# nabeelre/BTSbot

Hardware: AMD Instinct MI355X
Metric: alerts/sec (63×63×3 triplet + 25 meta) train+infer, 1/2/4/8 MI355X (higher is better)
Workload: dtype bf16; 1 GPU; BASELINE.json configs[1]: ConvNeXt-pico multi-modal (mm_ConvNeXt) bf16 inference, batch=1024 synthetic triplets per GPU, inputs resident in HBM, logits+scores out; per_gpu_batch=1024, global_batch=1024, precision=bf16, weights=seeded random, layer-scale ~1, parallelism=1 independent replicas, batch-sharded, no collective, pipeline_depth=3

## Files before the change

### btsbot_amd/csrc/stage0b.hip

```cpp
#include <type_traits>

#include "common.h"
#include "stage0.h"

namespace {

typedef __attribute__((ext_vector_type(16))) float f32x16;
typedef __attribute__((address_space(1))) const void* gptr_t;
typedef __attribute__((address_space(3))) void* lptr_t;

template <typename T> struct SBM;
typedef __attribute__((ext_vector_type(4))) short s16x4;
typedef __attribute__((ext_vector_type(4))) _Float16 f16x4;
template <> struct SBM<bf16_t> {
  using frag = bf16x8;
  using frag4 = s16x4;
  static __device__ __forceinline__ f32x16 run(frag a, frag b, f32x16 c) {
    return __builtin_amdgcn_mfma_f32_32x32x16_bf16(a, b, c, 0, 0, 0);
  }
  static __device__ __forceinline__ f32x4 run4(frag4 a, frag4 b, f32x4 c) {
    return __builtin_amdgcn_mfma_f32_4x4x4bf16_1k(a, b, c, 0, 0, 0);
  }
};
template <> struct SBM<f16_t> {
  using frag = f16x8;
  using frag4 = f16x4;
  static __device__ __forceinline__ f32x16 run(frag a, frag b, f32x16 c) {
    return __builtin_amdgcn_mfma_f32_32x32x16_f16(a, b, c, 0, 0, 0);
  }
  static __device__ __forceinline__ f32x4 run4(frag4 a, frag4 b, f32x4 c) {
    return __builtin_amdgcn_mfma_f32_4x4x4f16(a, b, c, 0, 0, 0);
  }
};

constexpr int C = 64, HW = 15, P = 225, CT = 2, HID = 256;
constexpr int PITCH = 2 * C + 16;
static_assert(256 * PITCH <= C * 800, "the [pixel][channel] image overlays the planar one");
constexpr int PL_ROWS = 22, PL_XQ = PL_ROWS * 8, PL_CH = 800;
constexpr int PLB = C * PL_CH;
constexpr int CHUNKB = 8192, NCH = HID / 32, NSLOT = 3;
constexpr int RINGB = NSLOT * CHUNKB;
constexpr int TW_R = 21, TW_BYTES = TW_R * C * 4 * 4 * 2;
constexpr int PF_DWB = 0, PF_LNW = C, PF_LNB = 2 * C, PF_B1 = 3 * C, PF_B2 = PF_B1 + HID, PF_FLOATS = 512;
static_assert(PF_B2 + C == PF_FLOATS, "parameter image layout");
constexpr int PARB = TW_BYTES + PF_FLOATS * 4;
constexpr int PARB_X2 = 2 * TW_BYTES + PF_FLOATS * 4;
template <bool X2> struct S0L {
  static constexpr int PLANES = X2 ? 2 : 1;
  static constexpr int CHB = X2 ? 2 * CHUNKB : CHUNKB;
  static constexpr int OFF_RING = PLANES * PLB;
  static constexpr int OFF_B1 = OFF_RING + NSLOT * CHB;
  static constexpr int OFF_ST = OFF_B1 + (HID + C) * 4;
  static constexpr int LDS_BYTES = OFF_ST + 2 * 256 * 4;
};
static_assert(S0L<false>::LDS_BYTES <= 81920, "two workgroups per CU");
static_assert(S0L<true>::LDS_BYTES <= 160 * 1024, "one workgroup per CU");
constexpr float LN_EPS = 1e-6f;

#define SB_STAMP(i)                                                                \
  do {                                                                             \
    if (a.stamps != nullptr && blockIdx.x == 0 && threadIdx.x == 0) {             \
      a.stamps[i] = clock64();                                                     \
      asm volatile("s_waitcnt vmcnt(0)" ::: "memory");  \
    }                                                                              \
    if (a.wgt != nullptr && threadIdx.x == 0 && ((i) == 0 || (i) == 13))           \
      a.wgt[2 * blockIdx.x + ((i) == 13)] = wall_clock64();                        \
  } while (0)

struct __attribute__((packed, aligned(4))) f4u { float v[4]; };

template <int N> __device__ __forceinline__ void wait_vm() {
  asm volatile("s_waitcnt vmcnt(%0)" ::"n"(N) : "memory");
}
__device__ __forceinline__ int swz4(int row) {
  return (4 - ((row >> 2) & 3)) & 3;
}
__device__ __forceinline__ float swap_add32(float a, float b) {
  auto r = __builtin_amdgcn_permlane32_swap(__float_as_uint(a), __float_as_uint(b), false, false);
  return __uint_as_float(r[0]) + __uint_as_float(r[1]);
}
__device__ __forceinline__ float swap_add16(float a, float b) {
  auto r = __builtin_amdgcn_permlane16_swap(__float_as_uint(a), __float_as_uint(b), false, false);
  return __uint_as_float(r[0]) + __uint_as_float(r[1]);
}
__device__ __forceinline__ void ln_regs(const f32x16 (&x)[CT], const float* __restrict__ w,
                                        const float* __restrict__ b, int h, f32x16 (&y)[CT]) {
  float s = 0.f;
#pragma unroll
  for (int ct = 0; ct < CT; ++ct)
#pragma unroll
    for (int r = 0; r < 16; ++r) s += x[ct][r];
  s += __shfl_xor(s, 32, 64);
  const float mean = s * (1.0f / C);
  float q = 0.f;
#pragma unroll
  for (int ct = 0; ct < CT; ++ct)
#pragma unroll
    for (int r = 0; r < 16; ++r) {
      const float d = x[ct][r] - mean;
      q += d * d;
    }
  q += __shfl_xor(q, 32, 64);
  const float rstd = rsqrtf(q * (1.0f / C) + LN_EPS);
#pragma unroll
  for (int ct = 0; ct < CT; ++ct)
#pragma unroll
    for (int qd = 0; qd < 4; ++qd) {
      const int c = ct * 32 + 8 * qd + 4 * h;
      const float4 wv = *reinterpret_cast<const float4*>(w + c);
      const float4 bv = *reinterpret_cast<const float4*>(b + c);
      y[ct][4 * qd + 0] = (x[ct][4 * qd + 0] - mean) * rstd * wv.x + bv.x;
      y[ct][4 * qd + 1] = (x[ct][4 * qd + 1] - mean) * rstd * wv.y + bv.y;
      y[ct][4 * qd + 2] = (x[ct][4 * qd + 2] - mean) * rstd * wv.z + bv.z;
      y[ct][4 * qd + 3] = (x[ct][4 * qd + 3] - mean) * rstd * wv.w + bv.w;
    }
}

template <typename T, int LOPLANE = 0>
__device__ __forceinline__ void regs_to_map(const f32x16 (&x)[CT], unsigned char* map, int p, int h) {
  typedef T T4 __attribute__((ext_vector_type(4)));
#pragma unroll
  for (int ct = 0; ct < CT; ++ct)
#pragma unroll
    for (int qd = 0; qd < 4; ++qd) {
      T4 v, w;
#pragma unroll
      for (int e = 0; e < 4; ++e) {
        v[e] = (T)x[ct][4 * qd + e];
        if (LOPLANE > 0) w[e] = (T)(x[ct][4 * qd + e] - (float)v[e]);
      }
      *reinterpret_cast<T4*>(map + p * PITCH + (ct * 32 + 8 * qd + 4 * h) * 2) = v;
      if (LOPLANE > 0) *reinterpret_cast<T4*>(map + LOPLANE + p * PITCH + (ct * 32 + 8 * qd + 4 * h) * 2) = w;
    }
}

template <typename T, int LOPLANE = 0, bool SAT = false>
__device__ __forceinline__ void regs_to_planar(const f32x16 (&x)[CT], unsigned char* pl, int p, int h) {
  const int y = p / HW, xx = p - y * HW;
  unsigned char* dst = pl + (xx >> 2) * PL_XQ + (y + 3) * 8 + (xx & 3) * 2 + h * 4 * PL_CH;
#pragma unroll
  for (int ct = 0; ct < CT; ++ct)
#pragma unroll
    for (int r = 0; r < 16; ++r) {
      const T hi = (T)(SAT ? __builtin_amdgcn_fmed3f(x[ct][r], -65504.0f, 65504.0f) : x[ct][r]);
      *reinterpret_cast<T*>(dst + (ct * 32 + 8 * (r >> 2) + (r & 3)) * PL_CH) = hi;
      if (LOPLANE > 0)
        *reinterpret_cast<T*>(dst + LOPLANE + (ct * 32 + 8 * (r >> 2) + (r & 3)) * PL_CH) = (T)(x[ct][r] - (float)hi);
    }
}

__device__ __forceinline__ void regs_to_tap(const f32x16 (&x)[CT], float* tap, int h) {
#pragma unroll
  for (int ct = 0; ct < CT; ++ct)
#pragma unroll
    for (int qd = 0; qd < 4; ++qd)
      *reinterpret_cast<float4*>(tap + ct * 32 + 8 * qd + 4 * h) =
          make_float4(x[ct][4 * qd], x[ct][4 * qd + 1], x[ct][4 * qd + 2], x[ct][4 * qd + 3]);
}

template <int CTRL> __device__ __forceinline__ float dpp_mov(float v) {
  return __builtin_bit_cast(float, __builtin_amdgcn_update_dpp(0, __builtin_bit_cast(int, v), CTRL, 0xF, 0xF, true));
}

template <bool SQ> __device__ __forceinline__ void block_reduce64(const float (&v)[64], int lane, float (&out)[4]) {
  float w[32];
#pragma unroll
  for (int n = 0; n < 32; ++n)
    w[n] = SQ ? swap_add32(v[n] * v[n], v[n + 32] * v[n + 32]) : swap_add32(v[n], v[n + 32]);
#pragma unroll
  for (int n = 0; n < 16; ++n) w[n] = swap_add16(w[n], w[n + 16]);
  const bool b3 = (lane & 8) != 0, b2 = (lane & 4) != 0;
#pragma unroll
  for (int n = 0; n < 8; ++n) {
    const float own = b3 ? w[n + 8] : w[n], send = b3 ? w[n] : w[n + 8];
    w[n] = own + dpp_mov<0x128>(send);
  }
#pragma unroll
  for (int n = 0; n < 4; ++n) {
    const float own = b2 ? w[n + 4] : w[n], send = b2 ? w[n] : w[n + 4];
    const float lo = dpp_mov<0x124>(send), hi = dpp_mov<0x12C>(send);
    out[n] = own + (b2 ? lo : hi);
  }
}

template <typename T, bool X2, int WPS = 2, bool KEEP = false>
__global__ __launch_bounds__(256, WPS) void stage0b_kernel(Stage0Args a) {
  using frag = typename SBM<T>::frag;
  using DT = typename std::conditional<KEEP, f16_t, T>::type;
  using frag4 = typename SBM<DT>::frag4;
  extern __shared__ __attribute__((aligned(16))) unsigned char smem[];
  unsigned char* map = smem;
  unsigned char* pl = smem;
  using L = S0L<X2>;
  constexpr int CHB = L::CHB;
  constexpr int PLO = X2 ? PLB : 0;
  unsigned char* ring = smem + L::OFF_RING;
  float* b1s = reinterpret_cast<float*>(smem + L::OFF_B1);
  float* b2s = b1s + HID;
  float* part = reinterpret_cast<float*>(ring + 2 * CHB);
  float* st = reinterpret_cast<float*>(smem + L::OFF_ST);

  const int tid = threadIdx.x, lane = tid & 63, wave = tid >> 6;
  const int lr = lane & 31, h = lane >> 5;
  const int alert = blockIdx.x;
  int pix[2];
  bool live[2];
#pragma unroll
  for (int t = 0; t < 2; ++t) {
    pix[t] = wave * 64 + t * 32 + lr;
    live[t] = pix[t] < P;
  }
  const int dj = lane & 3, dch = wave * 16 + (lane >> 2);
  const int dyb = lane >> 4, dxb = (lane >> 2) & 3;

  SB_STAMP(0);
  frag4 tw[TW_R], twl[X2 ? TW_R : 1];
  float dwbias, lng, lnb2, b1v, b2v;
  auto load_block_params = [&](int j) {
    const Stage0Blk& bk = a.blk[j];
    const uint2* src = reinterpret_cast<const uint2*>(bk.par) + wave * 64 + lane;
#pragma unroll
    for (int r = 0; r < TW_R; ++r) tw[r] = __builtin_bit_cast(frag4, src[r * 256]);
    if (X2) {
#pragma unroll
      for (int r = 0; r < TW_R; ++r) twl[r] = __builtin_bit_cast(frag4, src[TW_BYTES / 8 + r * 256]);
    }
    const float* pf = reinterpret_cast<const float*>(bk.par + (X2 ? 2 : 1) * TW_BYTES);
    dwbias = pf[PF_DWB + dch];
    lng = pf[PF_LNW + dch];
    lnb2 = pf[PF_LNB + dch];
    b1v = pf[PF_B1 + tid];
    b2v = pf[PF_B2 + (tid & 63)];
  };
  load_block_params(0);
  auto zero_planar = [&]() {
    for (int i = tid; i < L::PLANES * PLB / 16; i += 256) reinterpret_cast<uint4*>(pl)[i] = make_uint4(0u, 0u, 0u, 0u);
  };
  zero_planar();
  __syncthreads();

  f32x16 x[2][CT];
  {
    const float* src = a.img + (size_t)alert * 3 * 63 * 63;
    const T* sw = reinterpret_cast<const T*>(a.stem_w);
    frag af[3][CT], afl[X2 ? 3 : 1][CT];
#pragma unroll
    for (int ci = 0; ci < 3; ++ci)
#pragma unroll
      for (int ct = 0; ct < CT; ++ct) {
        af[ci][ct] = *reinterpret_cast<const frag*>(sw + (ct * 32 + lr) * 48 + ci * 16 + h * 8);
        if (X2)
          afl[ci][ct] = *reinterpret_cast<const frag*>(reinterpret_cast<const T*>(a.stem_w_lo) + (ct * 32 + lr) * 48 + ci * 16 + h * 8);
      }
#pragma unroll
    for (int t = 0; t < 2; ++t) {
      const int pc = live[t] ? pix[t] : 0;
      const int py = pc / HW, px = pc - py * HW;
#pragma unroll
      for (int ct = 0; ct < CT; ++ct)
#pragma unroll
        for (int qd = 0; qd < 4; ++qd) {
          const float4 bv = *reinterpret_cast<const float4*>(a.stem_b + ct * 32 + 8 * qd + 4 * h);
          x[t][ct][4 * qd + 0] = bv.x;
          x[t][ct][4 * qd + 1] = bv.y;
          x[t][ct][4 * qd + 2] = bv.z;
          x[t][ct][4 * qd + 3] = bv.w;
        }
#pragma unroll
      for (int ci = 0; ci < 3; ++ci) {
        const float* r0 = src + (ci * 63 + 4 * py + 2 * h) * 63 + 4 * px;
        const f4u v0 = *reinterpret_cast<const f4u*>(r0);
        const f4u v1 = *reinterpret_cast<const f4u*>(r0 + 63);
        frag bf, bfl;
#pragma unroll
        for (int e = 0; e < 4; ++e) {
          bf[e] = (T)v0.v[e];
          bf[4 + e] = (T)v1.v[e];
          if (X2) {
            bfl[e] = (T)(v0.v[e] - (float)bf[e]);
            bfl[4 + e] = (T)(v1.v[e] - (float)bf[4 + e]);
          }
        }
#pragma unroll
        for (int ct = 0; ct < CT; ++ct) {
          if (X2) {
            x[t][ct] = SBM<T>::run(afl[ci][ct], bf, x[t][ct]);
            x[t][ct] = SBM<T>::run(af[ci][ct], bfl, x[t][ct]);
          }
          x[t][ct] = SBM<T>::run(af[ci][ct], bf, x[t][ct]);
        }
      }
      if (KEEP && live[t]) regs_to_tap(x[t], a.keep_stem_pre + ((size_t)alert * P + pix[t]) * C, h);
      ln_regs(x[t], a.stem_lnw, a.stem_lnb, h, x[t]);
      if (live[t]) regs_to_planar<DT, PLO, KEEP && !std::is_same<T, f16_t>::value>(x[t], pl, pix[t], h);
      if (a.tap_stem != nullptr && live[t])
        regs_to_tap(x[t], a.tap_stem + ((size_t)alert * P + pix[t]) * C, h);
    }
  }
  SB_STAMP(1);

#pragma unroll
  for (int j = 0; j < 2; ++j) {
    const Stage0Blk& bk = a.blk[j];
    SB_STAMP(2 + 5 * j);
    __syncthreads();
    b1s[tid] = b1v;
    if (tid < C) b2s[tid] = b2v;

    const unsigned char* wsrc[2];
    const unsigned char* wsrcl[2];
#pragma unroll
    for (int i = 0; i < 2; ++i) {
      const int pc = wave * 2 + i;
      if (pc < 4) {
        const int m = pc * 8 + (lane >> 3);
        const int hid = (m & ~12) | ((m & 4) << 1) | ((m & 8) >> 1);
        const size_t o = (size_t)hid * (C * 2) + (((lane & 7) ^ ((m >> 1) & 7)) << 4);
        wsrc[i] = bk.w1 + o;
        wsrcl[i] = X2 ? bk.w1_lo + o : nullptr;
      } else {
        const int r = (pc - 4) * 16 + (lane >> 2);
        const size_t o = (size_t)r * (HID * 2) + (((lane & 3) ^ swz4(r)) << 4);
        wsrc[i] = bk.w2g + o;
        wsrcl[i] = X2 ? bk.w2g_lo + o : nullptr;
      }
    }
    const int wstep0 = wave < 2 ? 32 * C * 2 : 64;
    auto issue = [&](int ch) {
#pragma unroll
      for (int i = 0; i < 2; ++i)
        __builtin_amdgcn_global_load_lds((gptr_t)(wsrc[i] + (size_t)ch * wstep0),
                                         (lptr_t)(ring + (ch % NSLOT) * CHB + (wave * 2 + i) * 1024),
                                         16, 0, 0);
      if (X2) {
#pragma unroll
        for (int i = 0; i < 2; ++i)
          __builtin_amdgcn_global_load_lds((gptr_t)(wsrcl[i] + (size_t)ch * wstep0),
                                           (lptr_t)(ring + (ch % NSLOT) * CHB + CHUNKB + (wave * 2 + i) * 1024),
                                           16, 0, 0);
      }
    };
    SB_STAMP(3 + 5 * j);

    float v[64];
    {
      f32x4 acc[4][4];
#pragma unroll
      for (int yb = 0; yb < 4; ++yb)
#pragma unroll
        for (int xb = 0; xb < 4; ++xb) acc[yb][xb] = f32x4{dwbias, dwbias, dwbias, dwbias};
      const unsigned char* lb = pl + dch * PL_CH + dj * 8;
      frag4 bq[2][4], bql[X2 ? 2 : 1][X2 ? 4 : 1];
      auto read_step = [&](int s, int buf) {
#pragma unroll
        for (int q = 0; q < 4; ++q) {
          bq[buf][q] = __builtin_bit_cast(frag4, *reinterpret_cast<const uint2*>(lb + q * PL_XQ + s * 8));
          if (X2) bql[buf][q] = __builtin_bit_cast(frag4, *reinterpret_cast<const uint2*>(lb + PLB + q * PL_XQ + s * 8));
        }
      };
      read_step(0, 0);
#ifdef S0_EXP_NODW
#pragma unroll 1
      for (int s = 0; s < 1; ++s) {
#else
#pragma unroll
      for (int s = 0; s < 19; ++s) {
#endif
#pragma unroll
        for (int q = 0; q < 4; ++q) {
          asm volatile("" : "+v"(bq[s & 1][q]));
          if (X2) asm volatile("" : "+v"(bql[X2 ? s & 1 : 0][X2 ? q : 0]));
        }
        if (s + 1 < 19) read_step(s + 1, (s + 1) & 1);
        if (s == 0) {
          __builtin_amdgcn_sched_barrier(0);
          issue(0);
          issue(1);
        }
        __builtin_amdgcn_sched_barrier(0);
#pragma unroll
        for (int yb = 0; yb < 4; ++yb) {
          const int ky = s - 4 * yb;
          if (ky < 0 || ky > 6) continue;
#pragma unroll
          for (int rbi = 0; rbi < 3; ++rbi)
#pragma unroll
            for (int xb = 0; xb < 4; ++xb) {
              const int q = xb + rbi - 1;
              if (q < 0 || q > 3) continue;
              if (X2) {
                acc[yb][xb] = SBM<DT>::run4(twl[ky * 3 + rbi], bq[s & 1][q], acc[yb][xb]);
                acc[yb][xb] = SBM<DT>::run4(tw[ky * 3 + rbi], bql[X2 ? s & 1 : 0][X2 ? q : 0], acc[yb][xb]);
              }
              acc[yb][xb] = SBM<DT>::run4(tw[ky * 3 + rbi], bq[s & 1][q], acc[yb][xb]);
            }
        }
        __builtin_amdgcn_sched_barrier(0);
      }
#pragma unroll
      for (int yb = 0; yb < 4; ++yb)
#pragma unroll
        for (int xb = 0; xb < 4; ++xb)
#pragma unroll
          for (int i = 0; i < 4; ++i) v[yb * 16 + xb * 4 + i] = acc[yb][xb][i];
    }
    if (KEEP && a.keep_d[j] != nullptr) {
      float* dst = a.keep_d[j] + (size_t)alert * P * C + dch;
#pragma unroll
      for (int yb = 0; yb < 4; ++yb)
#pragma unroll
        for (int xb = 0; xb < 4; ++xb)
          if (yb < 3 || dj < 3) {
#pragma unroll
            for (int i = 0; i < 4; ++i) {
              if (xb == 3 && i == 3) continue;
              dst[((4 * yb + dj) * HW + 4 * xb + i) * C] = v[yb * 16 + xb * 4 + i];
            }
          }
    }
    SB_STAMP(4 + 5 * j);
    {
      float s1[4], s2[4];
#ifdef S0_EXP_NOLNRED
      for (int i = 0; i < 4; ++i) { s1[i] = v[i]; s2[i] = v[i + 4] * v[i + 4] + 1.f; }
#else
      block_reduce64<false>(v, lane, s1);
      block_reduce64<true>(v, lane, s2);
#endif
      const int slot = (4 * dyb + dj) * 16 + 4 * dxb;
      *reinterpret_cast<float4*>(part + wave * 256 + slot) = make_float4(s1[0], s1[1], s1[2], s1[3]);
      *reinterpret_cast<float4*>(part + 1024 + wave * 256 + slot) = make_float4(s2[0], s2[1], s2[2], s2[3]);
    }
    if (j == 0) SB_STAMP(14);
    __syncthreads();
    if (j == 0) SB_STAMP(15);
    {
      const float t1 = part[tid] + part[256 + tid] + part[512 + tid] + part[768 + tid];
      const float t2 = part[1024 + tid] + part[1280 + tid] + part[1536 + tid] + part[1792 + tid];
      const float mean = t1 * (1.0f / C);
      const float rstd = rsqrtf(fmaxf(t2 * (1.0f / C) - mean * mean, 0.0f) + LN_EPS);
      st[tid] = rstd;
      st[256 + tid] = -mean * rstd;
    }
    __syncthreads();
    auto write_ln = [&](bool lo_pass) {
      T* mo = reinterpret_cast<T*>(map) + dch;
#pragma unroll
      for (int yb = 0; yb < 4; ++yb)
#pragma unroll
        for (int xb = 0; xb < 4; ++xb) {
          const int slot = (4 * yb + dj) * 16 + 4 * xb;
          const float4 r4 = *reinterpret_cast<const float4*>(st + slot);
          const float4 m4 = *reinterpret_cast<const float4*>(st + 256 + slot);
          const float rr[4] = {r4.x, r4.y, r4.z, r4.w}, mm[4] = {m4.x, m4.y, m4.z, m4.w};
          if (yb < 3 || dj < 3) {
#pragma unroll
            for (int i = 0; i < 4; ++i) {
              if (xb == 3 && i == 3) continue;
              const float y = fmaf(fmaf(v[yb * 16 + xb * 4 + i], rr[i], mm[i]), lng, lnb2);
              const T yh = (T)y;
              mo[((4 * yb + dj) * HW + 4 * xb + i) * (PITCH / 2)] = lo_pass ? (T)(y - (float)yh) : yh;
            }
          }
        }
    };
    write_ln(false);
    SB_STAMP(5 + 5 * j);
    __syncthreads();
    if (KEEP) {
      unsigned char* dst = reinterpret_cast<unsigned char*>(a.keep_xn[j]) + (size_t)alert * P * C * 2;
      for (int i = tid; i < P * 8; i += 256) {
        const int p = i >> 3, c16 = i & 7;
        *reinterpret_cast<uint4*>(dst + (size_t)p * C * 2 + 16 * c16) = *reinterpret_cast<const uint4*>(map + p * PITCH + 16 * c16);
      }
    }

    {
      frag xf[2][4], xfl[X2 ? 2 : 1][4];
#pragma unroll
      for (int t = 0; t < 2; ++t)
#pragma unroll
        for (int ks = 0; ks < 4; ++ks)
          xf[t][ks] = *reinterpret_cast<const frag*>(map + pix[t] * PITCH + ks * 32 + h * 16);
      if (X2) {
        __syncthreads();
        write_ln(true);
        __syncthreads();
#pragma unroll
        for (int t = 0; t < 2; ++t)
#pragma unroll
          for (int ks = 0; ks < 4; ++ks)
            xfl[t][ks] = *reinterpret_cast<const frag*>(map + pix[t] * PITCH + ks * 32 + h * 16);
      }
#pragma unroll
      for (int ct = 0; ct < CT; ++ct)
#pragma unroll
        for (int qd = 0; qd < 4; ++qd) {
          const float4 bv = *reinterpret_cast<const float4*>(b2s + ct * 32 + 8 * qd + 4 * h);
#pragma unroll
          for (int t = 0; t < 2; ++t) {
            x[t][ct][4 * qd + 0] += bv.x;
            x[t][ct][4 * qd + 1] += bv.y;
            x[t][ct][4 * qd + 2] += bv.z;
            x[t][ct][4 * qd + 3] += bv.w;
          }
        }
#ifdef S0_EXP_NOLOOP
#pragma unroll 1
      for (int ch = 0; ch < 0; ++ch) {
#else
#pragma unroll 1
      for (int ch = 0; ch < NCH; ++ch) {
#endif
        if (ch + 1 < NCH) wait_vm<X2 ? 4 : 2>();
        else wait_vm<0>();
        asm volatile("s_waitcnt lgkmcnt(0)" ::: "memory");
        __builtin_amdgcn_s_barrier();
        if (ch == 1 && j == 0) zero_planar();
        const unsigned char* w1s = ring + (ch % NSLOT) * CHB;
        const unsigned char* w2s = w1s + 4096;
        frag a1[4], a2[CT][2], a1l[X2 ? 4 : 1], a2l[X2 ? CT : 1][2];
#pragma unroll
        for (int ks = 0; ks < 4; ++ks) {
          a1[ks] = *reinterpret_cast<const frag*>(w1s + lr * 128 + (((ks * 2 + h) ^ ((lr >> 1) & 7)) << 4));
          if (X2) a1l[ks] = *reinterpret_cast<const frag*>(w1s + CHUNKB + lr * 128 + (((ks * 2 + h) ^ ((lr >> 1) & 7)) << 4));
        }
#pragma unroll
        for (int ct = 0; ct < CT; ++ct)
#pragma unroll
          for (int s2 = 0; s2 < 2; ++s2) {
            const int r = ct * 32 + lr;
            a2[ct][s2] = *reinterpret_cast<const frag*>(w2s + r * 64 + (((s2 * 2 + h) ^ swz4(r)) << 4));
            if (X2) a2l[ct][s2] = *reinterpret_cast<const frag*>(w2s + CHUNKB + r * 64 + (((s2 * 2 + h) ^ swz4(r)) << 4));
          }
        f32x4 bq[4];
        {
          const unsigned baddr = (unsigned)(size_t)(lptr_t)(b1s + ch * 32 + 8 * h);
          asm volatile("ds_read_b128 %0, %4\n\tds_read_b128 %1, %4 offset:16\n\tds_read_b128 %2, %4 offset:64\n\t"
                       "ds_read_b128 %3, %4 offset:80\n\ts_waitcnt lgkmcnt(0)"
                       : "=&v"(bq[0]), "=&v"(bq[1]), "=&v"(bq[2]), "=&v"(bq[3]) : "v"(baddr) : "memory");
        }
        __builtin_amdgcn_sched_barrier(0);
        f32x16 hacc[2];
#pragma unroll
        for (int t = 0; t < 2; ++t) {
#pragma unroll
          for (int qd = 0; qd < 4; ++qd)
#pragma unroll
            for (int e = 0; e < 4; ++e) hacc[t][4 * qd + e] = bq[qd][e];
#pragma unroll
          for (int ks = 0; ks < 4; ++ks) {
            if (X2) {
              hacc[t] = SBM<T>::run(a1l[ks], xf[t][ks], hacc[t]);
              hacc[t] = SBM<T>::run(a1[ks], xfl[t][ks], hacc[t]);
            }
            hacc[t] = SBM<T>::run(a1[ks], xf[t][ks], hacc[t]);
          }
        }
        if (ch + 2 < NCH) issue(ch + 2);
#pragma unroll
        for (int t = 0; t < 2; ++t) {
#pragma unroll
          for (int s2 = 0; s2 < 2; ++s2) {
            frag hf, hfl;
#pragma unroll
            for (int r = 0; r < 8; ++r) {
#ifdef S0_EXP_NOGELU
              const float gv = hacc[t][8 * s2 + r];
#else
              const float gv = gelu_for<T>(hacc[t][8 * s2 + r]);
#endif
              hf[r] = (T)gv;
              if (X2) hfl[r] = (T)(gv - (float)hf[r]);
            }
#pragma unroll
            for (int ct = 0; ct < CT; ++ct) {
              if (X2) {
                x[t][ct] = SBM<T>::run(a2l[ct][s2], hf, x[t][ct]);
                x[t][ct] = SBM<T>::run(a2[ct][s2], hfl, x[t][ct]);
              }
              x[t][ct] = SBM<T>::run(a2[ct][s2], hf, x[t][ct]);
            }
          }
        }
      }
      if (j == 0) {
        load_block_params(1);
#pragma unroll
        for (int t = 0; t < 2; ++t) {
          if (live[t]) regs_to_planar<DT, PLO, KEEP && !std::is_same<T, f16_t>::value>(x[t], pl, pix[t], h);
          if (KEEP && live[t]) regs_to_tap(x[t], a.keep_xin1 + ((size_t)alert * P + pix[t]) * C, h);
        }
      }
    }
    SB_STAMP(6 + 5 * j);
  }
  if (a.tap_stage != nullptr) {
#pragma unroll
    for (int t = 0; t < 2; ++t)
      if (live[t]) regs_to_tap(x[t], a.tap_stage + ((size_t)alert * P + pix[t]) * C, h);
  }

  {
    const T* dw = reinterpret_cast<const T*>(a.ds_w) + (size_t)(wave * 32 + lr) * 256 + h * 8;
    frag af[16], afl[X2 ? 16 : 1];
#pragma unroll
    for (int ks = 0; ks < 16; ++ks) af[ks] = *reinterpret_cast<const frag*>(dw + ks * 16);
    constexpr int MAPB = 256 * PITCH;
    static_assert(2 * MAPB <= L::OFF_B1, "two [pixel][channel] images in front of the bias words");
    if (X2) __syncthreads();
#pragma unroll
    for (int t = 0; t < 2; ++t) {
      f32x16 xn[CT];
      ln_regs(x[t], a.ds_lnw, a.ds_lnb, h, xn);
      regs_to_map<T, X2 ? MAPB : 0>(xn, map, pix[t], h);
    }
    if (X2) {
      const T* dwl = reinterpret_cast<const T*>(a.ds_w_lo) + (size_t)(wave * 32 + lr) * 256 + h * 8;
#pragma unroll
      for (int ks = 0; ks < 16; ++ks) afl[ks] = *reinterpret_cast<const frag*>(dwl + ks * 16);
    }
    __syncthreads();
    if (KEEP) {
      unsigned char* dst = reinterpret_cast<unsigned char*>(a.keep_patches) + (size_t)alert * 49 * 4 * C * 2;
      for (int i = tid; i < 49 * 4 * 8; i += 256) {
        const int c16 = i & 7, q = (i >> 3) & 3, o = i >> 5;
        const int pin = (2 * (o / 7) + (q >> 1)) * HW + 2 * (o % 7) + (q & 1);
        *reinterpret_cast<uint4*>(dst + (size_t)(o * 4 + q) * C * 2 + 16 * c16) =
            *reinterpret_cast<const uint4*>(map + pin * PITCH + 16 * c16);
      }
    }
    SB_STAMP(12);
#pragma unroll
    for (int t = 0; t < 2; ++t) {
      const int o = t * 32 + lr;
      const bool olive = o < 49;
      const int oc = olive ? o : 0;
      const int oy = oc / 7, ox = oc - oy * 7;
      f32x16 acc;
#pragma unroll
      for (int qd = 0; qd < 4; ++qd) {
        const float4 bv = *reinterpret_cast<const float4*>(a.ds_b + wave * 32 + 8 * qd + 4 * h);
        acc[4 * qd + 0] = bv.x;
        acc[4 * qd + 1] = bv.y;
        acc[4 * qd + 2] = bv.z;
        acc[4 * qd + 3] = bv.w;
      }
#pragma unroll
      for (int ks = 0; ks < 16; ++ks) {
        const int q = ks >> 2;
        const int pin = (2 * oy + (q >> 1)) * HW + 2 * ox + (q & 1);
        const frag bf = *reinterpret_cast<const frag*>(map + pin * PITCH + (ks & 3) * 32 + h * 16);
        if (X2) {
          const frag bfl = *reinterpret_cast<const frag*>(map + MAPB + pin * PITCH + (ks & 3) * 32 + h * 16);
          acc = SBM<T>::run(afl[ks], bf, acc);
          acc = SBM<T>::run(af[ks], bfl, acc);
        }
        acc = SBM<T>::run(af[ks], bf, acc);
      }
      if (olive) {
        float* dst = a.out + ((size_t)alert * 49 + o) * 128 + wave * 32 + 4 * h;
#pragma unroll
        for (int qd = 0; qd < 4; ++qd)
          *reinterpret_cast<float4*>(dst + 8 * qd) =
              make_float4(acc[4 * qd], acc[4 * qd + 1], acc[4 * qd + 2], acc[4 * qd + 3]);
      }
    }
    SB_STAMP(13);
  }
}

template <typename T, bool X2>
__global__ void pack_s0par_kernel(const float* __restrict__ taps, const float* __restrict__ dw_b,
                                  const float* __restrict__ ln_w, const float* __restrict__ ln_b,
                                  const float* __restrict__ b1, const float* __restrict__ b2,
                                  const float* __restrict__ gamma, unsigned char* __restrict__ out) {
  const int idx = blockIdx.x * blockDim.x + threadIdx.x;
  constexpr int NTW = TW_R * C * 16;
  if (idx < NTW) {
    const int k = idx & 3, i = (idx >> 2) & 3, c = (idx >> 4) & (C - 1), r = idx >> 10;
    const int ky = r / 3, rb = r % 3 - 1, kx = 4 * rb + k - i + 3;
    const float w = (kx >= 0 && kx < 7) ? taps[(ky * 7 + kx) * C + c] : 0.f;
    const T wh = (T)w;
    reinterpret_cast<T*>(out)[idx] = wh;
    if (X2) reinterpret_cast<T*>(out)[NTW + idx] = (T)(w - (float)wh);
    return;
  }
  const int f = idx - NTW;
  if (f >= PF_FLOATS) return;
  float v;
  if (f < PF_LNW) v = dw_b[f - PF_DWB];
  else if (f < PF_LNB) v = ln_w[f - PF_LNW];
  else if (f < PF_B1) v = ln_b[f - PF_LNB];
  else if (f < PF_B2) v = b1[f - PF_B1];
  else v = gamma[f - PF_B2] * b2[f - PF_B2];
  reinterpret_cast<float*>(out + (X2 ? 2 : 1) * TW_BYTES)[f] = v;
}

template <typename T, bool X2 = false, int WPS = 2, bool KEEP = false> int launch_stage0b_t(const Stage0Args& a, hipStream_t st) {
  auto kern = stage0b_kernel<T, X2, WPS, KEEP>;
  static DevOnce attr_set;
  static const int pad = switch_on(SW_S0_ONE_WG) && !X2 ? 90 * 1024 - S0L<X2>::LDS_BYTES : 0;
  const int LDS_BYTES = S0L<X2>::LDS_BYTES + pad;
  if (attr_set.need()) {
    HIP_TRY(hipFuncSetAttribute(reinterpret_cast<const void*>(kern),
                                hipFuncAttributeMaxDynamicSharedMemorySize, (int)LDS_BYTES));
    attr_set.done();
  }
  hipLaunchKernelGGL(kern, dim3(a.B), dim3(256), LDS_BYTES, st, a);
  LAUNCH_CHECK();
  return BTSBOT_OK;
}

}

#ifdef STAGE0B_X2_TU
int launch_stage0b_x2(const Stage0Args& a, hipStream_t st) {
  return launch_stage0b_t<f16_t, true, 1>(a, st);
}
int launch_pack_s0par_x2(const float* taps, const float* dw_b, const float* ln_w, const float* ln_b, const float* b1,
                         const float* b2, const float* gamma, void* out, hipStream_t st) {
  const dim3 grid((TW_R * C * 16 + PF_FLOATS + 255) / 256), blk(256);
  hipLaunchKernelGGL((pack_s0par_kernel<f16_t, true>), grid, blk, 0, st, taps, dw_b, ln_w, ln_b, b1, b2, gamma,
                     reinterpret_cast<unsigned char*>(out));
  LAUNCH_CHECK();
  return BTSBOT_OK;
}
#else
int launch_stage0b_x2(const Stage0Args& a, hipStream_t st);
int launch_pack_s0par_x2(const float* taps, const float* dw_b, const float* ln_w, const float* ln_b, const float* b1,
                         const float* b2, const float* gamma, void* out, hipStream_t st);

size_t s0par_bytes() { return PARB_X2; }

int launch_pack_s0par(int prec, const float* taps, const float* dw_b, const float* ln_w, const float* ln_b,
                      const float* b1, const float* b2, const float* gamma, void* out, hipStream_t st) {
  const dim3 grid((TW_R * C * 16 + PF_FLOATS + 255) / 256), blk(256);
  unsigned char* o = reinterpret_cast<unsigned char*>(out);
  if (prec == BTSBOT_BF16)
    hipLaunchKernelGGL((pack_s0par_kernel<bf16_t, false>), grid, blk, 0, st, taps, dw_b, ln_w, ln_b, b1, b2, gamma, o);
  else if (prec == BTSBOT_F16)
    hipLaunchKernelGGL((pack_s0par_kernel<f16_t, false>), grid, blk, 0, st, taps, dw_b, ln_w, ln_b, b1, b2, gamma, o);
  else if (prec == BTSBOT_F16X2)
    return launch_pack_s0par_x2(taps, dw_b, ln_w, ln_b, b1, b2, gamma, out, st);
  else {
    btsbot_set_error("pack_s0par: precision %d is not a 16-bit mode", prec);
    return BTSBOT_ERR_INVALID_ARG;
  }
  LAUNCH_CHECK();
  return BTSBOT_OK;
}

bool stage0_supported(int prec, int c0) {
  return (prec == BTSBOT_BF16 || prec == BTSBOT_F16 || prec == BTSBOT_F16X2) && c0 == 64;
}

int launch_stage0b(int prec, const Stage0Args& a, hipStream_t st) {
  if (a.B <= 0) return BTSBOT_OK;
  if (a.keep_xn[0] != nullptr) {
    if (a.keep_stem_pre == nullptr || a.tap_stem == nullptr || a.keep_xin1 == nullptr || a.tap_stage == nullptr ||
        (a.keep_d[0] == nullptr) != (a.keep_d[1] == nullptr) || a.keep_xn[1] == nullptr || a.keep_patches == nullptr) {
      btsbot_set_error("stage0b: the training forward needs every kept buffer");
      return BTSBOT_ERR_INVALID_ARG;
    }
    if (prec == BTSBOT_BF16) return launch_stage0b_t<bf16_t, false, 2, true>(a, st);
    if (prec == BTSBOT_F16) return launch_stage0b_t<f16_t, false, 2, true>(a, st);
    btsbot_set_error("stage0b: the training forward runs in the bf16 / f16 modes, not %d", prec);
    return BTSBOT_ERR_INVALID_ARG;
  }
  if (prec == BTSBOT_BF16) return launch_stage0b_t<bf16_t>(a, st);
  if (prec == BTSBOT_F16) return launch_stage0b_t<f16_t>(a, st);
  if (prec == BTSBOT_F16X2) {
    if (a.ds_w_lo == nullptr || a.stem_w_lo == nullptr || a.blk[0].w1_lo == nullptr || a.blk[0].w2g_lo == nullptr ||
        a.blk[1].w1_lo == nullptr || a.blk[1].w2g_lo == nullptr) {
      btsbot_set_error("stage0b: the split mode needs the remainder images (ds_w_lo, stem_w_lo, w1_lo, w2g_lo)");
      return BTSBOT_ERR_INVALID_ARG;
    }
    return launch_stage0b_x2(a, st);
  }
  btsbot_set_error("stage0b: unsupported precision %d", prec);
  return BTSBOT_ERR_INVALID_ARG;
}
#endif
```

Measured before the change: 3.460 million alerts/s.

## Compute stage-0 LayerNorm per pixel from an fp32 LDS image instead of cross-lane reductions

```diff
diff --git a/btsbot_amd/csrc/stage0b.hip b/btsbot_amd/csrc/stage0b.hip
--- a/btsbot_amd/csrc/stage0b.hip
+++ b/btsbot_amd/csrc/stage0b.hip
@@ -39,22 +39,26 @@
 constexpr int PL_ROWS = 22, PL_XQ = PL_ROWS * 8, PL_CH = 800;
 constexpr int PLB = C * PL_CH;
 constexpr int CHUNKB = 8192, NCH = HID / 32, NSLOT = 3;
-constexpr int RINGB = NSLOT * CHUNKB;
 constexpr int TW_R = 21, TW_BYTES = TW_R * C * 4 * 4 * 2;
 constexpr int PF_DWB = 0, PF_LNW = C, PF_LNB = 2 * C, PF_B1 = 3 * C, PF_B2 = PF_B1 + HID, PF_FLOATS = 512;
 static_assert(PF_B2 + C == PF_FLOATS, "parameter image layout");
 constexpr int PARB = TW_BYTES + PF_FLOATS * 4;
 constexpr int PARB_X2 = 2 * TW_BYTES + PF_FLOATS * 4;
+constexpr int LNP = 4 * C + 16;
+constexpr int LNIMGB = P * LNP;
+static_assert(LNIMGB % 16 == 0 && PLB + CHUNKB <= LNIMGB, "ring slot 2 inside the image's tail, behind the planar image");
 template <bool X2> struct S0L {
   static constexpr int PLANES = X2 ? 2 : 1;
   static constexpr int CHB = X2 ? 2 * CHUNKB : CHUNKB;
-  static constexpr int OFF_RING = PLANES * PLB;
-  static constexpr int OFF_B1 = OFF_RING + NSLOT * CHB;
-  static constexpr int OFF_ST = OFF_B1 + (HID + C) * 4;
-  static constexpr int LDS_BYTES = OFF_ST + 2 * 256 * 4;
+  static constexpr int OFF_RING = X2 ? PLANES * PLB : LNIMGB;
+  static constexpr int OFF_SLOT2 = X2 ? OFF_RING + 2 * CHB : PLB;
+  static constexpr int OFF_B1 = OFF_RING + (X2 ? NSLOT : 2) * CHB;
+  static constexpr int LDS_BYTES = OFF_B1 + (HID + 3 * C) * 4;
+  static __device__ __forceinline__ int slot(int s) { return s == 2 ? OFF_SLOT2 : OFF_RING + s * CHB; }
 };
 static_assert(S0L<false>::LDS_BYTES <= 81920, "two workgroups per CU");
 static_assert(S0L<true>::LDS_BYTES <= 160 * 1024, "one workgroup per CU");
+static_assert(LNIMGB <= S0L<true>::OFF_RING && LNIMGB <= S0L<false>::OFF_RING, "the fp32 image in front of ring slots 0 and 1");
 constexpr float LN_EPS = 1e-6f;
 
 #define SB_STAMP(i)                                                                \
@@ -75,14 +79,6 @@
 __device__ __forceinline__ int swz4(int row) {
   return (4 - ((row >> 2) & 3)) & 3;
 }
-__device__ __forceinline__ float swap_add32(float a, float b) {
-  auto r = __builtin_amdgcn_permlane32_swap(__float_as_uint(a), __float_as_uint(b), false, false);
-  return __uint_as_float(r[0]) + __uint_as_float(r[1]);
-}
-__device__ __forceinline__ float swap_add16(float a, float b) {
-  auto r = __builtin_amdgcn_permlane16_swap(__float_as_uint(a), __float_as_uint(b), false, false);
-  return __uint_as_float(r[0]) + __uint_as_float(r[1]);
-}
 __device__ __forceinline__ void ln_regs(const f32x16 (&x)[CT], const float* __restrict__ w,
                                         const float* __restrict__ b, int h, f32x16 (&y)[CT]) {
   float s = 0.f;
@@ -156,31 +152,6 @@
     for (int qd = 0; qd < 4; ++qd)
       *reinterpret_cast<float4*>(tap + ct * 32 + 8 * qd + 4 * h) =
           make_float4(x[ct][4 * qd], x[ct][4 * qd + 1], x[ct][4 * qd + 2], x[ct][4 * qd + 3]);
-}
-
-template <int CTRL> __device__ __forceinline__ float dpp_mov(float v) {
-  return __builtin_bit_cast(float, __builtin_amdgcn_update_dpp(0, __builtin_bit_cast(int, v), CTRL, 0xF, 0xF, true));
-}
-
-template <bool SQ> __device__ __forceinline__ void block_reduce64(const float (&v)[64], int lane, float (&out)[4]) {
-  float w[32];
-#pragma unroll
-  for (int n = 0; n < 32; ++n)
-    w[n] = SQ ? swap_add32(v[n] * v[n], v[n + 32] * v[n + 32]) : swap_add32(v[n], v[n + 32]);
-#pragma unroll
-  for (int n = 0; n < 16; ++n) w[n] = swap_add16(w[n], w[n + 16]);
-  const bool b3 = (lane & 8) != 0, b2 = (lane & 4) != 0;
-#pragma unroll
-  for (int n = 0; n < 8; ++n) {
-    const float own = b3 ? w[n + 8] : w[n], send = b3 ? w[n] : w[n + 8];
-    w[n] = own + dpp_mov<0x128>(send);
-  }
-#pragma unroll
-  for (int n = 0; n < 4; ++n) {
-    const float own = b2 ? w[n + 4] : w[n], send = b2 ? w[n] : w[n + 4];
-    const float lo = dpp_mov<0x124>(send), hi = dpp_mov<0x12C>(send);
-    out[n] = own + (b2 ? lo : hi);
-  }
 }
 
 template <typename T, bool X2, int WPS = 2, bool KEEP = false>
@@ -192,13 +163,11 @@
   unsigned char* map = smem;
   unsigned char* pl = smem;
   using L = S0L<X2>;
-  constexpr int CHB = L::CHB;
   constexpr int PLO = X2 ? PLB : 0;
-  unsigned char* ring = smem + L::OFF_RING;
   float* b1s = reinterpret_cast<float*>(smem + L::OFF_B1);
   float* b2s = b1s + HID;
-  float* part = reinterpret_cast<float*>(ring + 2 * CHB);
-  float* st = reinterpret_cast<float*>(smem + L::OFF_ST);
+  float* lnws = b2s + C;
+  float* lnbs = lnws + C;
 
   const int tid = threadIdx.x, lane = tid & 63, wave = tid >> 6;
   const int lr = lane & 31, h = lane >> 5;
@@ -211,7 +180,6 @@
     live[t] = pix[t] < P;
   }
   const int dj = lane & 3, dch = wave * 16 + (lane >> 2);
-  const int dyb = lane >> 4, dxb = (lane >> 2) & 3;
 
   SB_STAMP(0);
   frag4 tw[TW_R], twl[X2 ? TW_R : 1];
@@ -227,8 +195,8 @@
     }
     const float* pf = reinterpret_cast<const float*>(bk.par + (X2 ? 2 : 1) * TW_BYTES);
     dwbias = pf[PF_DWB + dch];
-    lng = pf[PF_LNW + dch];
-    lnb2 = pf[PF_LNB + dch];
+    lng = pf[PF_LNW + (tid & 63)];
+    lnb2 = pf[PF_LNB + (tid & 63)];
     b1v = pf[PF_B1 + tid];
     b2v = pf[PF_B2 + (tid & 63)];
   };
@@ -305,7 +273,11 @@
     SB_STAMP(2 + 5 * j);
     __syncthreads();
     b1s[tid] = b1v;
-    if (tid < C) b2s[tid] = b2v;
+    if (tid < C) {
+      b2s[tid] = b2v;
+      lnws[tid] = lng;
+      lnbs[tid] = lnb2;
+    }
 
     const unsigned char* wsrc[2];
     const unsigned char* wsrcl[2];
@@ -330,13 +302,13 @@
 #pragma unroll
       for (int i = 0; i < 2; ++i)
         __builtin_amdgcn_global_load_lds((gptr_t)(wsrc[i] + (size_t)ch * wstep0),
-                                         (lptr_t)(ring + (ch % NSLOT) * CHB + (wave * 2 + i) * 1024),
+                                         (lptr_t)(smem + L::slot(ch % NSLOT) + (wave * 2 + i) * 1024),
                                          16, 0, 0);
       if (X2) {
 #pragma unroll
         for (int i = 0; i < 2; ++i)
           __builtin_amdgcn_global_load_lds((gptr_t)(wsrcl[i] + (size_t)ch * wstep0),
-                                           (lptr_t)(ring + (ch % NSLOT) * CHB + CHUNKB + (wave * 2 + i) * 1024),
+                                           (lptr_t)(smem + L::slot(ch % NSLOT) + CHUNKB + (wave * 2 + i) * 1024),
                                            16, 0, 0);
       }
     };
@@ -419,79 +391,75 @@
           }
     }
     SB_STAMP(4 + 5 * j);
+    __syncthreads();
     {
-      float s1[4], s2[4];
-#ifdef S0_EXP_NOLNRED
-      for (int i = 0; i < 4; ++i) { s1[i] = v[i]; s2[i] = v[i + 4] * v[i + 4] + 1.f; }
-#else
-      block_reduce64<false>(v, lane, s1);
-      block_reduce64<true>(v, lane, s2);
-#endif
-      const int slot = (4 * dyb + dj) * 16 + 4 * dxb;
-      *reinterpret_cast<float4*>(part + wave * 256 + slot) = make_float4(s1[0], s1[1], s1[2], s1[3]);
-      *reinterpret_cast<float4*>(part + 1024 + wave * 256 + slot) = make_float4(s2[0], s2[1], s2[2], s2[3]);
+      float* dst = reinterpret_cast<float*>(smem + dj * HW * LNP) + dch;
+#pragma unroll
+      for (int yb = 0; yb < 4; ++yb)
+#pragma unroll
+        for (int xb = 0; xb < 4; ++xb)
+          if (yb < 3 || dj < 3) {
+#pragma unroll
+            for (int i = 0; i < 4; ++i) {
+              if (xb == 3 && i == 3) continue;
+              dst[(4 * yb * HW + 4 * xb + i) * (LNP / 4)] = v[yb * 16 + xb * 4 + i];
+            }
+          }
     }
     if (j == 0) SB_STAMP(14);
     __syncthreads();
     if (j == 0) SB_STAMP(15);
-    {
-      const float t1 = part[tid] + part[256 + tid] + part[512 + tid] + part[768 + tid];
-      const float t2 = part[1024 + tid] + part[1280 + tid] + part[1536 + tid] + part[1792 + tid];
-      const float mean = t1 * (1.0f / C);
-      const float rstd = rsqrtf(fmaxf(t2 * (1.0f / C) - mean * mean, 0.0f) + LN_EPS);
-      st[tid] = rstd;
-      st[256 + tid] = -mean * rstd;
-    }
-    __syncthreads();
-    auto write_ln = [&](bool lo_pass) {
-      T* mo = reinterpret_cast<T*>(map) + dch;
-#pragma unroll
-      for (int yb = 0; yb < 4; ++yb)
-#pragma unroll
-        for (int xb = 0; xb < 4; ++xb) {
-          const int slot = (4 * yb + dj) * 16 + 4 * xb;
-          const float4 r4 = *reinterpret_cast<const float4*>(st + slot);
-          const float4 m4 = *reinterpret_cast<const float4*>(st + 256 + slot);
-          const float rr[4] = {r4.x, r4.y, r4.z, r4.w}, mm[4] = {m4.x, m4.y, m4.z, m4.w};
-          if (yb < 3 || dj < 3) {
-#pragma unroll
-            for (int i = 0; i < 4; ++i) {
-              if (xb == 3 && i == 3) continue;
-              const float y = fmaf(fmaf(v[yb * 16 + xb * 4 + i], rr[i], mm[i]), lng, lnb2);
-              const T yh = (T)y;
-              mo[((4 * yb + dj) * HW + 4 * xb + i) * (PITCH / 2)] = lo_pass ? (T)(y - (float)yh) : yh;
-            }
-          }
-        }
-    };
-    write_ln(false);
-    SB_STAMP(5 + 5 * j);
-    __syncthreads();
-    if (KEEP) {
-      unsigned char* dst = reinterpret_cast<unsigned char*>(a.keep_xn[j]) + (size_t)alert * P * C * 2;
-      for (int i = tid; i < P * 8; i += 256) {
-        const int p = i >> 3, c16 = i & 7;
-        *reinterpret_cast<uint4*>(dst + (size_t)p * C * 2 + 16 * c16) = *reinterpret_cast<const uint4*>(map + p * PITCH + 16 * c16);
-      }
-    }
 
     {
       frag xf[2][4], xfl[X2 ? 2 : 1][4];
 #pragma unroll
-      for (int t = 0; t < 2; ++t)
+      for (int t = 0; t < 2; ++t) {
+        const unsigned char* row = smem + (live[t] ? pix[t] : P - 1) * LNP + h * 32;
+        float xv[32];
 #pragma unroll
         for (int ks = 0; ks < 4; ++ks)
-          xf[t][ks] = *reinterpret_cast<const frag*>(map + pix[t] * PITCH + ks * 32 + h * 16);
-      if (X2) {
-        __syncthreads();
-        write_ln(true);
-        __syncthreads();
-#pragma unroll
-        for (int t = 0; t < 2; ++t)
-#pragma unroll
-          for (int ks = 0; ks < 4; ++ks)
-            xfl[t][ks] = *reinterpret_cast<const frag*>(map + pix[t] * PITCH + ks * 32 + h * 16);
-      }
+#pragma unroll
+          for (int q = 0; q < 2; ++q) {
+            const float4 r4 = *reinterpret_cast<const float4*>(row + ks * 64 + q * 16);
+            xv[ks * 8 + q * 4 + 0] = r4.x;
+            xv[ks * 8 + q * 4 + 1] = r4.y;
+            xv[ks * 8 + q * 4 + 2] = r4.z;
+            xv[ks * 8 + q * 4 + 3] = r4.w;
+          }
+        float s = 0.f;
+#pragma unroll
+        for (int n = 0; n < 32; ++n) s += xv[n];
+        s += __shfl_xor(s, 32, 64);
+        const float mean = s * (1.0f / C);
+        float q2 = 0.f;
+#pragma unroll
+        for (int n = 0; n < 32; ++n) {
+          xv[n] -= mean;
+          q2 += xv[n] * xv[n];
+        }
+        q2 += __shfl_xor(q2, 32, 64);
+        const float rstd = rsqrtf(q2 * (1.0f / C) + LN_EPS);
+#pragma unroll
+        for (int ks = 0; ks < 4; ++ks) {
+#pragma unroll
+          for (int q = 0; q < 2; ++q) {
+            const float4 w4 = *reinterpret_cast<const float4*>(lnws + ks * 16 + h * 8 + q * 4);
+            const float4 b4 = *reinterpret_cast<const float4*>(lnbs + ks * 16 + h * 8 + q * 4);
+            const float ww[4] = {w4.x, w4.y, w4.z, w4.w}, bb[4] = {b4.x, b4.y, b4.z, b4.w};
+#pragma unroll
+            for (int e = 0; e < 4; ++e) {
+              const float y = xv[ks * 8 + q * 4 + e] * rstd * ww[e] + bb[e];
+              const T yh = (T)y;
+              xf[t][ks][q * 4 + e] = yh;
+              if (X2) xfl[t][ks][q * 4 + e] = (T)(y - (float)yh);
+            }
+          }
+          if (KEEP && live[t])
+            *reinterpret_cast<frag*>(reinterpret_cast<unsigned char*>(a.keep_xn[j]) +
+                                     ((size_t)alert * P + pix[t]) * C * 2 + ks * 32 + h * 16) = xf[t][ks];
+        }
+      }
+      SB_STAMP(5 + 5 * j);
 #pragma unroll
       for (int ct = 0; ct < CT; ++ct)
 #pragma unroll
@@ -517,7 +485,7 @@
         asm volatile("s_waitcnt lgkmcnt(0)" ::: "memory");
         __builtin_amdgcn_s_barrier();
         if (ch == 1 && j == 0) zero_planar();
-        const unsigned char* w1s = ring + (ch % NSLOT) * CHB;
+        const unsigned char* w1s = smem + L::slot(ch % NSLOT);
         const unsigned char* w2s = w1s + 4096;
         frag a1[4], a2[CT][2], a1l[X2 ? 4 : 1], a2l[X2 ? CT : 1][2];
 #pragma unroll
@@ -607,8 +575,7 @@
 #pragma unroll
     for (int ks = 0; ks < 16; ++ks) af[ks] = *reinterpret_cast<const frag*>(dw + ks * 16);
     constexpr int MAPB = 256 * PITCH;
-    static_assert(2 * MAPB <= L::OFF_B1, "two [pixel][channel] images in front of the bias words");
-    if (X2) __syncthreads();
+    static_assert(MAPB <= PLB && 2 * MAPB <= S0L<true>::OFF_RING, "the 16-bit [pixel][channel] image(s) in front of every ring slot");
 #pragma unroll
     for (int t = 0; t < 2; ++t) {
       f32x16 xn[CT];
```

Measured after the change: 3.639 million alerts/s, median of 6. 5.2% higher.
